# Yixin-F/better_fastlio2

Measured on NVIDIA H100. Metric: scans/s (120k-pt, 3 ESIKF iters) at 1xH100; kNN+Jacobian HBM GB/s vs peak, higher is better.
Workload: dtype f32 search/plane + f64 Jacobian/ESIKF

## Files before the change

better_fastlio2_b200/csrc/esikf_device.cuh:

```cuda
#pragma once
#include "meas_kernels.cuh"

namespace flb {

namespace dev {

constexpr int ESIKF_THREADS = 256;

__device__ __forceinline__ void qmul(const double* a, const double* b, double* r) {
  const double x = a[3] * b[0] + a[0] * b[3] + a[1] * b[2] - a[2] * b[1];
  const double y = a[3] * b[1] + a[1] * b[3] + a[2] * b[0] - a[0] * b[2];
  const double z = a[3] * b[2] + a[2] * b[3] + a[0] * b[1] - a[1] * b[0];
  const double w = a[3] * b[3] - a[0] * b[0] - a[1] * b[1] - a[2] * b[2];
  r[0] = x; r[1] = y; r[2] = z; r[3] = w;
}
__device__ __forceinline__ void rotmat(const double* q, double* R) {
  const double tx = 2 * q[0], ty = 2 * q[1], tz = 2 * q[2];
  const double twx = tx * q[3], twy = ty * q[3], twz = tz * q[3], txx = tx * q[0], txy = ty * q[0], txz = tz * q[0];
  const double tyy = ty * q[1], tyz = tz * q[1], tzz = tz * q[2];
  R[0] = 1 - (tyy + tzz); R[1] = txy - twz; R[2] = txz + twy;
  R[3] = txy + twz; R[4] = 1 - (txx + tzz); R[5] = tyz - twx;
  R[6] = txz - twy; R[7] = tyz + twx; R[8] = 1 - (txx + tyy);
}
__device__ __forceinline__ void hat(const double* v, double* H) {
// ... 172 lines not shown
  if (tid < PROJ_OUT) v = proj_row_value(M, NDOF, q, c);
  __syncthreads();
  if (tid < PROJ_OUT) M[(q.idx + q.i) * NDOF + c] = v;
  __syncthreads();
  if (tid < PROJ_OUT) v = proj_col_value(M, q, c);
  __syncthreads();
  if (tid < PROJ_OUT) M[c * NDOF + q.idx + q.i] = v;
  __syncthreads();
}
}

__global__ void k_esikf_begin(EsikfCtl* c, const double* __restrict__ stage, int* work_counts) {
  pdl_sync();
  FLB_TRACE_BEGIN(0);
  if (threadIdx.x == 0) c->t_begin = global_timer_ns();
  __shared__ double sst[26 + NDOF * NDOF + 4];
  constexpr int NPAIR = (26 + NDOF * NDOF + 4) / 2;
  const double2* st2 = reinterpret_cast<const double2*>(stage);
  for (int i = threadIdx.x; i < NPAIR; i += blockDim.x) {
    const double2 v = st2[i];
    sst[2 * i] = v.x;
    sst[2 * i + 1] = v.y;
  }
  if (threadIdx.x >= 32 && threadIdx.x < 48) work_counts[threadIdx.x - 32] = 0;
  __syncthreads();
  const double* x0 = sst;
  const double* P0 = sst + 26;
  const int n = (int)sst[26 + NDOF * NDOF];
  for (int i = threadIdx.x; i < NDOF * NDOF; i += blockDim.x) { c->Pp[i] = P0[i]; c->P[i] = P0[i]; }
  if (threadIdx.x < 26) { c->x[threadIdx.x] = x0[threadIdx.x]; c->xp[threadIdx.x] = x0[threadIdx.x]; }
  __syncthreads();
  if (threadIdx.x == 0) {
    c->it = -1; c->t = 0; c->converge = 1; c->finished = 0; c->need_host = 0; c->passes = 0; c->searches = 0;
    c->lastM = 0; c->last_res = 0.0; c->n = n; c->flg_inited = (int)sst[26 + NDOF * NDOF + 1];
    c->body = reinterpret_cast<const float4*>((unsigned long long)__double_as_longlong(sst[26 + NDOF * NDOF + 2]));
    dev::pose_from_state(c->x, c->pose);
  }
  FLB_TRACE_END(0);
}

struct StepResult {
  double x[26];
  double P[NDOF * NDOF];
  double last_res;
  int passes, searches, lastM, t, need_host, pad_;
  int counters[32];
  int cnt2[2];
// ... 281 lines not shown
```

better_fastlio2_b200/csrc/fastlio_b200.cu:

```cuda
#include "../../include/fastlio_b200.h"
#include "map_kernels.cuh"
#include "knn_kernels.cuh"
#include "frontend_kernels.cuh"
#include "meas_kernels.cuh"
#include "esikf_device.cuh"
#include "knn_tile.cuh"
#include "esikf_host.hpp"

#include <cub/device/device_scan.cuh>
#include <algorithm>
#include <chrono>
#include <climits>
#include <cstdarg>
#include <cstdio>
#include <cstdlib>
#include <cstring>
#include <new>
#include <vector>

using namespace flb;

static thread_local char g_err[512] = "";
static int set_err(const char* fmt, ...) {
  va_list ap;
// ... 33 lines not shown
template <typename T> using DevBuf = GrowBuf<T, false>;
template <typename T> using PinnedBuf = GrowBuf<T, true>;

template <typename T, bool Pinned>
static int grow(GrowBuf<T, Pinned>& b, size_t need, size_t floor) {
  if (need <= b.cap) return 0;
  b.release();
  const size_t cap = std::max(need, floor);
  void* p = nullptr;
  CU(Pinned ? cudaMallocHost(&p, cap) : cudaMalloc(&p, cap));
  b.p = static_cast<T*>(p);
  b.cap = cap;
  return 0;
}

extern "C" const char* flb_last_error(void) { return g_err; }
extern "C" const char* flb_version(void) { return "fastlio_b200 0.1 (sm_90a)"; }
extern "C" int flb_device_count(void) {
  int n = 0;
  if (cudaGetDeviceCount(&n) != cudaSuccess) { cudaGetLastError(); return 0; }
  return n;
}

static bool pdl_enabled() {
  static const bool on = [] { const char* e = getenv("FLB_PDL"); return e && atoi(e) != 0; }();
  return on;
}
template <typename... P, typename... A>
static cudaError_t launch_k(void (*kern)(P...), dim3 grid, dim3 block, size_t smem, cudaStream_t st, A&&... args) {
  cudaLaunchConfig_t cfg{};
  cfg.gridDim = grid; cfg.blockDim = block; cfg.dynamicSmemBytes = smem; cfg.stream = st;
  cudaLaunchAttribute at[1];
  at[0].id = cudaLaunchAttributeProgrammaticStreamSerialization;
  at[0].val.programmaticStreamSerializationAllowed = 1;
  cfg.attrs = at;
  cfg.numAttrs = pdl_enabled() ? 1 : 0;
  return cudaLaunchKernelEx(&cfg, kern, static_cast<P>(args)...);
}

static inline uint32_t next_pow2(uint64_t v) {
  uint32_t p = 1;
  while (p < v) p <<= 1;
  return p;
}
static inline int grid_for(int n, int threads, int max_blocks) {
  int g = (n + threads - 1) / threads;
  if (g < 1) g = 1;
  return g > max_blocks ? max_blocks : g;
}
template <typename... P>
static cudaError_t resident_ctas(void (*kern)(P...), int threads, size_t smem, int sm_count, int& out) {
  int per_sm = 0;
  const cudaError_t e = cudaOccupancyMaxActiveBlocksPerMultiprocessor(&per_sm, kern, threads, smem);
  out = std::max(per_sm, 1) * sm_count;
  return e;
}

struct flb_map {
  MapDev d{};
  flb_map_config cfg{};
// ... 71 lines not shown
  m->has_root = false;
  return 0;
}

static int absorb_range_flag(flb_map* m) {
  int e = m->h_counters[CNT_ERROR];
  if (!(e & ERR_RANGE)) return e;
  if (!m->warned_range) {
    fprintf(stderr, "[fastlio_b200] warning: point(s) outside the representable range / NaN were skipped by the map insert\n");
    m->warned_range = true;
  }
  e &= ~ERR_RANGE;
  m->h_counters[CNT_ERROR] = e;
  if (cudaMemcpyAsync(m->d.counters + CNT_ERROR, m->h_counters + CNT_ERROR, sizeof(int), cudaMemcpyHostToDevice, m->stream) == cudaSuccess)
    cudaStreamSynchronize(m->stream);
  return e;
}

static int fetch_counters(flb_map* m) {
  CU(cudaMemcpyAsync(m->h_counters, m->d.counters, sizeof(int) * CNT_COUNT, cudaMemcpyDeviceToHost, m->stream));
  CU(cudaStreamSynchronize(m->stream));
  const int e = absorb_range_flag(m);
  if (e) {
    return set_err("device map error flags 0x%x:%s%s%s%s%s", e, (e & ERR_BLOCKS_FULL) ? " block pool exhausted (raise max_blocks)" : "",
                   (e & ERR_OVF_FULL) ? " overflow pool exhausted (raise max_points)" : "", (e & ERR_HASH_FULL) ? " block hash full" : "",
                   (e & ERR_COARSE_FULL) ? " coarse hash full" : "", (e & ERR_RANGE) ? " point outside representable range / NaN" : "");
  }
  return 0;
}

extern "C" int flb_map_create(const flb_map_config* cfg, flb_map** out) {
  if (!cfg || !out) return set_err("flb_map_create: null argument");
  cudaGetLastError();
  if (!(cfg->voxel_size > 0.f)) return set_err("flb_map_create: voxel_size must be > 0");
  int ndev = flb_device_count();
  if (ndev <= 0) return set_err("flb_map_create: no CUDA device available (this library has no CPU fallback)");
  if (cfg->device < 0 || cfg->device >= ndev) return set_err("flb_map_create: bad device %d", cfg->device);
  CU(cudaSetDevice(cfg->device));
  flb_map* m = new (std::nothrow) flb_map();
  if (!m) return set_err("out of host memory");
  m->cfg = *cfg;
  if (m->cfg.max_points <= 0) m->cfg.max_points = 8 * 1024 * 1024;
  if (m->cfg.max_blocks <= 0) m->cfg.max_blocks = std::max(4096, m->cfg.max_points / 4);
  cudaDeviceProp prop;
  CU(cudaGetDeviceProperties(&prop, cfg->device));
  m->sm_count = prop.multiProcessorCount;
  CU(resident_ctas(k_knn<5>, KNN_THREADS, 0, m->sm_count, m->exact_ctas[0]));
  CU(resident_ctas(k_knn<20>, KNN_THREADS, 0, m->sm_count, m->exact_ctas[1]));
  CU(cudaStreamCreateWithFlags(&m->stream, cudaStreamNonBlocking));
  MapDev& d = m->d;
  d.ds = cfg->voxel_size;
  d.block_cap = m->cfg.max_blocks;
  d.ovf_cap = std::max(1024, m->cfg.max_points / 2);
  m->hash_cap = next_pow2((uint64_t)d.block_cap * 4);
  m->chash_cap = next_pow2(std::max<uint64_t>(1024, (uint64_t)d.block_cap / 8));
  d.hash_mask = m->hash_cap - 1;
  d.chash_mask = m->chash_cap - 1;
  int rc = 0;
  rc |= dev_alloc(m, (void**)&d.hent, sizeof(HEntry) * m->hash_cap);
  rc |= dev_alloc(m, (void**)&d.bslot, sizeof(uint32_t) * d.block_cap);
  rc |= dev_alloc(m, (void**)&d.slots, sizeof(float4) * 64 * (size_t)d.block_cap);
  rc |= dev_alloc(m, (void**)&d.ovf, sizeof(float4) * (size_t)d.ovf_cap);
  rc |= dev_alloc(m, (void**)&d.sint, sizeof(float) * 64 * (size_t)d.block_cap);
  rc |= dev_alloc(m, (void**)&d.oint, sizeof(float) * (size_t)d.ovf_cap);
  rc |= dev_alloc(m, (void**)&d.bkey, sizeof(uint64_t) * d.block_cap);
  rc |= dev_alloc(m, (void**)&d.brel, sizeof(uint64_t) * d.block_cap);
  rc |= dev_alloc(m, (void**)&d.free_blk, sizeof(uint32_t) * d.block_cap);
  rc |= dev_alloc(m, (void**)&d.free_ovf, sizeof(uint32_t) * d.ovf_cap);
  rc |= dev_alloc(m, (void**)&d.ckeys, sizeof(uint64_t) * m->chash_cap);
  rc |= dev_alloc(m, (void**)&d.cbits, sizeof(uint64_t) * 8 * (size_t)m->chash_cap);
  rc |= dev_alloc(m, (void**)&d.clist, sizeof(uint32_t) * (size_t)m->chash_cap);
  rc |= dev_alloc(m, (void**)&d.counters, sizeof(int) * CNT_COUNT);
  rc |= dev_alloc(m, (void**)&m->d_misc, sizeof(int) * 32);
  rc |= dev_alloc(m, (void**)&m->d_phase, sizeof(int) * 8);
  if (rc) { flb_map_destroy(m); return 1; }
  if (cudaMallocHost((void**)&m->h_counters, sizeof(int) * CNT_COUNT) != cudaSuccess) { flb_map_destroy(m); return set_err("cudaMallocHost failed"); }
  unsigned char ti[91], tj[91];
  int e = 0;
  for (int i = 0; i < 13; ++i) for (int j = i; j < 13; ++j) { ti[e] = (unsigned char)i; tj[e] = (unsigned char)j; ++e; }
  CU(cudaMemcpyToSymbol(c_tri_i, ti, sizeof(ti)));
  CU(cudaMemcpyToSymbol(c_tri_j, tj, sizeof(tj)));
  if (map_reset_storage(m)) { flb_map_destroy(m); return 1; }
  *out = m;
  return 0;
}

static void map_release(flb_map* m);
static void kfw_release(KfWork* w);
extern "C" void flb_map_destroy(flb_map* m) {
  if (!m) return;
  map_release(m);
}
static void map_release(flb_map* m) {
  if (--m->refs > 0) return;
  Q(cudaSetDevice(m->cfg.device));
  if (m->stream) Q(cudaStreamSynchronize(m->stream));
// ... 43 lines not shown
  return pack_records(m, st, raw.p, n, stride, off_i, off_c, dst, curv);
}

static int upload_points(flb_map* m, const void* pts, int n, int stride, int off_i = -1) {
  if (n <= 0) return 0;
  if (!pts) return set_err("null point buffer");
  if (stride < 12) return set_err("stride_bytes must be >= 12");
  if (off_i >= 0 && off_i + 4 > stride) return set_err("intensity offset %d outside the %d-byte record", off_i, stride);
  if (stride == 16 && off_i < 0) off_i = 12;
  if (grow(m->stage, sizeof(float4) * (size_t)n, sizeof(float4) << 16)) return 1;
  return upload_records(m, m->stream, m->raw, (size_t)1 << 20, pts, n, stride, off_i, -1, m->stage.p, nullptr);
}

static inline uint32_t scratch_slots(int n) { return next_pow2((uint64_t)std::max(n, 512) * 2); }

static int ensure_scratch(flb_map* m, int n) {
  const size_t need = sizeof(uint64_t) * scratch_slots(n);
  if (need <= m->skeys.cap && need <= m->sbest.cap) return 0;
  if (grow(m->skeys, need, 0) || grow(m->sbest, need, 0)) return 1;
  m->gen++;
  return 0;
}

static int ensure_worklist(flb_map* m, int n) {
  const size_t need = sizeof(int) * (size_t)n;
  if (need <= m->worklist.cap) return 0;
  if (grow(m->worklist, need, sizeof(int) << 17)) return 1;
  m->gen++;
  return 0;
}

static int maybe_rehash(flb_map* m);

static int insert_device(flb_map* m, const float4* pts, const unsigned char* cls, int n, int mode, const int* skip = nullptr,
                         const int* n_dev = nullptr, bool prefused = false, StepTail tail = StepTail{}) {
  if (n <= 0) return 0;
  const int g = grid_for(n, 256, m->sm_count * 8);
  cudaStream_t st = m->stream;
  const unsigned char* c = (mode == 2) ? cls : nullptr;
  ProfScope ps(m, FLB_K_INSERT);
  if (!prefused) {
    launch_k(k_touch_blocks, g, 256, 0, st, m->d, pts, c, (1 << 1) | (1 << 2), n, skip, n_dev);
    m->launches++;
  }
  if (mode == 1 || mode == 2) {
    const uint32_t sc = scratch_slots(n);
    if (!prefused) {
      if (ensure_scratch(m, n)) return 1;
      if (!m->scratch_clean) {
        CU(cudaMemsetAsync(m->skeys.p, 0xFF, sizeof(uint64_t) * sc, st));
// ... 113 lines not shown
  m->launches += 2;
  CU(cudaMemsetAsync(m->d.ckeys, 0xFF, sizeof(uint64_t) * m->chash_cap, st));
  CU(cudaMemsetAsync(m->d.cbits, 0, sizeof(uint64_t) * 8 * (size_t)m->chash_cap, st));
  int init[8] = {0, 0, INT_MAX, INT_MAX, INT_MAX, INT_MIN, INT_MIN, INT_MIN};
  CU(cudaMemcpyAsync(m->d.counters + CNT_KEYS_TOMB, &init[0], sizeof(int), cudaMemcpyHostToDevice, st));
  CU(cudaMemcpyAsync(m->d.counters + CNT_COARSE_USED, &init[1], sizeof(int), cudaMemcpyHostToDevice, st));
  CU(cudaMemcpyAsync(m->d.counters + CNT_CMIN_X, &init[2], sizeof(int) * 6, cudaMemcpyHostToDevice, st));
  CU(cudaStreamSynchronize(st));
  k_rehash_insert<<<grid_for(nblk, 256, m->sm_count * 8), 256, 0, st>>>(m->d, nblk);
  m->launches++;
  CU(cudaGetLastError());
  m->rehash_count++;
  return fetch_counters(m);
}

template <int K>
static int launch_knn(flb_map* m, KnnArgs a) {
  if (ensure_worklist(m, a.n)) return 1;
  a.worklist = m->worklist.p;
  if (a.stride <= 0) a.stride = a.n;
  if (!a.work_count) {
    a.work_count = m->d_misc + 12;
    a.work_ticket = m->d_misc + 13;
    CU(cudaMemsetAsync(a.work_count, 0, 2 * sizeof(int), m->stream));
  }
  launch_k(k_knn_stencil<K>, (a.n + 127) / 128, 128, 0, m->stream, a);
  launch_k(k_knn<K>, m->exact_ctas[K == 5 ? 0 : 1], KNN_THREADS, 0, m->stream, a);
  m->launches += 2;
  return 0;
}

static int ensure_outbuf(flb_map* m, int n) { return grow(m->outbuf, sizeof(float4) * (size_t)n, sizeof(float4) << 16); }

static int nearest_search_impl(flb_map* m, const float* q_xyz, int nq, int stride, int k, float max_dist, float* out_pts, int out_w,
                               float* out_d2, int* out_cnt) {
  if (!m) return set_err("null map");
  if (k < 1 || k > 20) return set_err("Nearest_Search: k must be in [1,20]");
  if (nq <= 0) return 0;
  CU(cudaSetDevice(m->cfg.device));
  if (upload_points(m, q_xyz, nq, stride)) return 1;
  const int K = k <= 5 ? 5 : 20;
  if (ensure_outbuf(m, nq * K)) return 1;
  unsigned char* dcnt = nullptr;
  float* dint = nullptr;
  CU(cudaMalloc((void**)&dcnt, nq));
  KnnArgs a;
  a.m = m->d; a.q = m->stage.p; a.n = nq; a.nbr = m->outbuf.p; a.cnt = dcnt;
  a.max_d2 = (max_dist > 0.f && max_dist < 1e18f) ? max_dist * max_dist : INFINITY;
  a.phase_stats = nullptr;
  a.ctl = nullptr; a.body = nullptr; a.stride = nq; a.work_count = nullptr;
// ... 166 lines not shown
    float ms = 0.f;
    if (cudaEventElapsedTime(&ms, r.a, r.b) != cudaSuccess) continue;
    if (r.cls >= 0 && r.cls < FLB_K_COUNT) { out->ms[r.cls] += ms; out->launches[r.cls] += r.nlaunch; out->regions[r.cls] += 1; }
  }
  int ph[8];
  CU(cudaMemcpy(ph, m->d_phase, sizeof(ph), cudaMemcpyDeviceToHost));
  for (int i = 0; i < 4; ++i) out->knn_phase[i] = ph[i];
  out->knn_chain_nodes = ph[4]; out->knn_chain_max = ph[5]; out->knn_head_candidates = ph[6];
  if (reset) { m->prof_used = 0; CU(cudaMemset(m->d_phase, 0, sizeof(int) * 8)); }
  return 0;
}

extern "C" int flb_debug_knn_bench(flb_map* m, const float* q_xyz, int nq, int stride, int variant, int iters, float* ms_per_launch,
                                   int* unresolved, float* out_d2, int* out_cnt) {
  if (!m || !q_xyz || nq <= 0 || iters <= 0) return set_err("flb_debug_knn_bench: bad argument");
  CU(cudaSetDevice(m->cfg.device));
  if (upload_points(m, q_xyz, nq, stride)) return 1;
  if (ensure_outbuf(m, nq * 5)) return 1;
  if (ensure_worklist(m, nq)) return 1;
  unsigned char* dcnt = nullptr;
  CU(cudaMalloc((void**)&dcnt, nq));
  KnnArgs a;
  a.m = m->d; a.q = m->stage.p; a.n = nq; a.nbr = m->outbuf.p; a.cnt = dcnt; a.max_d2 = INFINITY; a.phase_stats = nullptr;
  a.worklist = m->worklist.p; a.work_count = m->d_misc + 12; a.work_ticket = m->d_misc + 13; a.ctl = nullptr; a.body = nullptr; a.stride = nq;
  cudaError_t e = cudaFuncSetAttribute(k_knn_tile<5>, cudaFuncAttributeMaxDynamicSharedMemorySize, (int)sizeof(TileSmem));
  cudaEvent_t e0 = nullptr, e1 = nullptr;
  if (e == cudaSuccess) e = cudaEventCreate(&e0);
  if (e == cudaSuccess) e = cudaEventCreate(&e1);
  const int grid = (nq + 127) / 128;
  for (int it = -2; it < iters && e == cudaSuccess; ++it) {
    if (it == 0) e = cudaEventRecord(e0, m->stream);
    if (e == cudaSuccess) e = cudaMemsetAsync(a.work_count, 0, 2 * sizeof(int), m->stream);
    if (variant == 0) k_knn_stencil<5><<<grid, 128, 0, m->stream>>>(a);
    else k_knn_tile<5><<<grid, TILE_THREADS, sizeof(TileSmem), m->stream>>>(a);
    if (e == cudaSuccess) e = cudaGetLastError();
  }
  if (e == cudaSuccess) e = cudaEventRecord(e1, m->stream);
  if (e == cudaSuccess) e = cudaStreamSynchronize(m->stream);
  float ms = 0.f;
  if (e == cudaSuccess) e = cudaEventElapsedTime(&ms, e0, e1);
  if (ms_per_launch) *ms_per_launch = ms / (float)iters;
  if (e == cudaSuccess && unresolved) e = cudaMemcpy(unresolved, a.work_count, sizeof(int), cudaMemcpyDeviceToHost);
  if (e == cudaSuccess && out_d2) {
    std::vector<float4> h((size_t)nq * 5);
    e = cudaMemcpy(h.data(), m->outbuf.p, sizeof(float4) * h.size(), cudaMemcpyDeviceToHost);
    for (int i = 0; i < nq && e == cudaSuccess; ++i)
      for (int j = 0; j < 5; ++j) out_d2[(size_t)i * 5 + j] = h[(size_t)j * nq + i].w;
  }
  if (e == cudaSuccess && out_cnt) {
    std::vector<unsigned char> hc(nq);
    e = cudaMemcpy(hc.data(), dcnt, nq, cudaMemcpyDeviceToHost);
    for (int i = 0; i < nq; ++i) out_cnt[i] = hc[i];
  }
  cudaFree(dcnt);
  if (e0) cudaEventDestroy(e0);
  if (e1) cudaEventDestroy(e1);
  if (e != cudaSuccess) return set_err("flb_debug_knn_bench: %s", cudaGetErrorString(e));
  return 0;
}

struct flb_session {
// ... 425 lines not shown
      if (md12) k_esikf_pre<12><<<1, dev::ESIKF_THREADS, 0, s->side>>>(s->ctl, s->d_scr);
      else k_esikf_pre<6><<<1, dev::ESIKF_THREADS, 0, s->side>>>(s->ctl, s->d_scr);
      if (p == 0 && with_insert) {
        if (!m->capturing && ensure_scratch(m, cap)) return 1;
        const uint32_t sc = scratch_slots(cap);
        CU(cudaMemsetAsync(m->skeys.p, 0xFF, sizeof(uint64_t) * sc, s->side));
        CU(cudaMemsetAsync(m->sbest.p, 0xFF, sizeof(unsigned long long) * sc, s->side));
        CU(cudaMemsetAsync(s->d_cnt2, 0, sizeof(int) * 2, s->side));
        m->scratch_clean = true;
      }
      CU(cudaEventRecord(s->ev_join[p], s->side));
    } else {
      ProfScope ps(m, FLB_K_REDUCE);
      if (md12) k_esikf_pre<12><<<1, dev::ESIKF_THREADS, 0, st>>>(s->ctl, s->d_scr);
      else k_esikf_pre<6><<<1, dev::ESIKF_THREADS, 0, st>>>(s->ctl, s->d_scr);
    }
    m->launches++;
    {
      ProfScope ps(m, FLB_K_KNN);
      KnnArgs a;
      a.m = m->d; a.q = nullptr; a.n = cap; a.nbr = s->nbr; a.cnt = s->cnt; a.max_d2 = INFINITY;
      a.phase_stats = m->prof_on ? m->d_phase : nullptr;
      a.ctl = s->ctl; a.body = nullptr; a.stride = cap; a.work_count = p < 8 ? m->d_misc + 16 + p : nullptr; a.work_ticket = p < 8 ? m->d_misc + 24 + p : nullptr;
      if (launch_knn<5>(m, a)) return 1;
    }
    {
      ProfScope ps(m, FLB_K_RESIDUAL);
      MeasArgs ma = meas_args(s, PoseDev{}, 0);
      ma.ctl = s->ctl;
      if (s->cfg.extrinsic_est_en) launch_k(k_residual<true>, s->res_grid, meas_threads<true>(), meas_smem_bytes<true>(), st, ma);
      else launch_k(k_residual<false>, s->res_grid, meas_threads<false>(), meas_smem_bytes<false>(), st, ma);
      m->launches++;
    }
    if (overlap) CU(cudaStreamWaitEvent(st, s->ev_join[p], 0));
    {
      ProfScope ps(m, FLB_K_REDUCE);
      if (md12) launch_k(k_esikf_post<12>, 1, dev::ESIKF_THREADS, 0, st, s->ctl, (const double*)s->partial, s->res_grid, s->d_scr);
      else launch_k(k_esikf_post<6>, 1, dev::ESIKF_THREADS, 0, st, s->ctl, (const double*)s->partial, s->res_grid, s->d_scr);
      m->launches++;
    }
  }
  CU(cudaGetLastError());
  const bool tail_publish = overlap && with_insert && s->cap > 0;
  if (tail_publish) {
    CU(cudaEventRecord(s->ev_fork[8], st));
    CU(cudaStreamWaitEvent(s->side, s->ev_fork[8], 0));
// ... 377 lines not shown
```

better_fastlio2_b200/csrc/knn_kernels.cuh:

```cuda
#pragma once
#include "mask_bits.h"
#include "voxel_map.cuh"
#include <math_constants.h>

namespace flb {

constexpr unsigned FULL = 0xffffffffu;
constexpr int BLOCK_RINGS = 8;
#ifndef FLB_KNN_THREADS
#define FLB_KNN_THREADS 128
#endif
#ifndef FLB_KNN_MINB
#define FLB_KNN_MINB 4
#endif
constexpr int KNN_THREADS = FLB_KNN_THREADS;
constexpr int KNN_MIN_CTAS = FLB_KNN_MINB;

__host__ __device__ constexpr int topk_unroll(int k) { return k <= 8 ? k : 1; }

template <int K>
struct TopK {
  float d[K], x[K], y[K], z[K];
  __device__ __forceinline__ void clear() {
#pragma unroll (topk_unroll(K))
// ... 112 lines not shown
  double limit[NDOF];
  double R;
  double last_res;
  PoseDev pose;
  int max_iter, it, t, converge, finished, need_host, passes, searches, lastM, n;
  int flg_inited;
  int pad_;
  const float4* body;
  unsigned long long t_begin;
};
__device__ __forceinline__ bool ctl_pass_active(const EsikfCtl* c) { return !c->finished && c->it < c->max_iter; }

struct KnnArgs {
  MapDev m;
  const float4* q;
  int n;
  float4* nbr;
  unsigned char* cnt;
  float max_d2;
  int* phase_stats;
  int* worklist;
  int* work_count;
  int* work_ticket;
  const EsikfCtl* ctl;
  const float4* body;
  int stride;
};

__device__ __forceinline__ float box_mind2(float qx, float qy, float qz, float lx, float ly, float lz, float hx, float hy, float hz, float mg) {
  const float gx = fmaxf(fmaxf(lx - qx, qx - hx) - mg, 0.f);
  const float gy = fmaxf(fmaxf(ly - qy, qy - hy) - mg, 0.f);
  const float gz = fmaxf(fmaxf(lz - qz, qz - hz) - mg, 0.f);
  return gx * gx + gy * gy + gz * gz;
}
__device__ __forceinline__ float cover2(float qx, float qy, float qz, float lx, float ly, float lz, float hx, float hy, float hz, float mg) {
  float c = fminf(fminf(fminf(qx - lx, hx - qx), fminf(qy - ly, hy - qy)), fminf(qz - lz, hz - qz)) - mg;
  return c > 0.f ? c * c : 0.f;
}

constexpr int EXACT_RINGS = 8;
constexpr int CAND_CAP = 512;

struct ExactSmem {
  unsigned cand[KNN_THREADS / 32][CAND_CAP];
  unsigned long long cbits[KNN_THREADS / 32][27 * 8];
};
// ... 232 lines not shown
#pragma unroll 1
        for (int base = 0; base < ncs; base += 32) {
          int cs;
          const float md = cell_md(base + lane, cs);
          const bool go = md > level && md < CUDART_INF_F && (wcount < K || md <= wthr) && md <= lim;
          unsigned todo = __ballot_sync(FULL, go);
          if (!todo) continue;
          while (todo) {
            const int c = __ffs(todo) - 1;
            todo &= todo - 1;
            scan_coarse_cell<K>(m, cand, cb, __shfl_sync(FULL, cs, c), lane, wqx, wqy, wqz, cvx, cvy, cvz, wcount == K, wthr, lim, mg, tw);
          }
          wcount = warp_merge<K>(tw, FULL, lane, lane, wd_, wx, wy, wz, wthr);
        }
      }
    }
    if (lane < K) nbr[(size_t)lane * stride + qi] = make_float4(wx, wy, wz, wd_);
    if (lane == 0) {
      cnt[qi] = (unsigned char)wcount;
      if (phase_stats) atomicAdd(&phase_stats[phase], 1);
    }
}

template <int K>
__global__ void __launch_bounds__(KNN_THREADS, KNN_MIN_CTAS) k_knn(KnnArgs a) {
  pdl_sync();
  __shared__ ExactSmem sm;
  const MapDev& m = a.m;
  const int lane = threadIdx.x & 31, wid = threadIdx.x >> 5;
  const float ds = m.ds;
  const float lim = a.max_d2;
  unsigned* cand = sm.cand[wid];
  unsigned long long* cb = sm.cbits[wid];
  FLB_TRACE_BEGIN(3 * 8 + (a.ctl ? a.ctl->it + 1 : 0));
  if (a.ctl && !(ctl_pass_active(a.ctl) && a.ctl->converge)) return;
  const int nwork = *a.work_count;
  const int nwarps = (int)(gridDim.x * (blockDim.x >> 5));
  int w = (int)(blockIdx.x * (blockDim.x >> 5)) + wid;
  for (;; ) {
    if (w >= nwork) break;
    const int i = a.worklist[w];
    const float4 q4 = a.ctl ? body_to_world(a.ctl->pose, __ldg(&a.ctl->body[i])) : __ldg(&a.q[i]);
    const float qx = q4.x, qy = q4.y, qz = q4.z;
    TopK<K> t;
    t.clear();
    float rd = CUDART_INF_F, rx = CUDART_NAN_F, ry = CUDART_NAN_F, rz = CUDART_NAN_F, thr = CUDART_INF_F;
    int gcount = a.cnt[i];
    if (lane < gcount) {
      const float4 sd = a.nbr[(size_t)lane * a.stride + i];
      rd = sd.w; rx = sd.x; ry = sd.y; rz = sd.z;
      t.d[0] = rd; t.x[0] = rx; t.y[0] = ry; t.z[0] = rz;
    }
    {
      const float dk = __shfl_sync(FULL, rd, K - 1);
      thr = gcount == K ? dk : CUDART_INF_F;
    }
    const int cvx = voxel_of(qx, ds), cvy = voxel_of(qy, ds), cvz = voxel_of(qz, ds);
    const float mg = 1e-3f * ds + 4.8e-7f * (fabsf(qx) + fabsf(qy) + fabsf(qz));
    const int qbx = cvx >> 2, qby = cvy >> 2, qbz = cvz >> 2;
    const int qcx = qbx >> 3, qcy = qby >> 3, qcz = qbz >> 3;
    const float bs4 = 4.f * ds;
    bool done = false;
    FLB_DBG_CLOCK(e0);
    int dbg_rings = 0;
    (void)dbg_rings;
#ifdef FLB_TRACE
    long long ph_probe = 0, ph_merge = 0, ph_mark = clock64();
    const long long ph_seed = ph_mark - e0;
#define KPH(acc) { const long long now_ = clock64(); acc += now_ - ph_mark; ph_mark = now_; }
#else
#define KPH(acc)
#endif
// ... 37 lines not shown
    if (done) {
      if (lane < K) a.nbr[(size_t)lane * a.stride + i] = make_float4(rx, ry, rz, rd);
      if (lane == 0) {
        a.cnt[i] = (unsigned char)gcount;
        if (a.phase_stats) atomicAdd(&a.phase_stats[1], 1);
      }
    }
#ifdef FLB_TRACE
    if (lane == 0 && a.ctl && a.ctl->it == -1) {
      const long long e1 = clock64();
      FLB_DBG_ADD(16, 1); FLB_DBG_ADD(17, e1 - e0); FLB_DBG_MAX(18, e1 - e0); FLB_DBG_ADD(18 + min(dbg_rings, 6), 1);
      FLB_DBG_ADD(25, done ? 0 : 1);
      FLB_DBG_ADD(58 + (int)min((e1 - e0) >> 13, 5ll), 1);
      FLB_DBG_ADD(32, ph_seed); FLB_DBG_ADD(33, ph_probe); FLB_DBG_ADD(36, ph_merge);
    }
#endif
    if (!done) {
      __syncwarp();
      warp_finish_coarse<K>(m, cand, cb, a.nbr, a.cnt, a.phase_stats, a.stride, lim, i, qx, qy, qz, gcount, thr, rd, rx, ry, rz);
    }
    if (lane == 0) w = nwarps + atomicAdd(a.work_ticket, 1);
    w = __shfl_sync(FULL, w, 0);
  }
  FLB_TRACE_END(3 * 8 + (a.ctl ? a.ctl->it + 1 : 0));
}

template <int K>
struct TopKId {
  float d[K];
  unsigned id[K];
  __device__ __forceinline__ void clear() {
#pragma unroll
    for (int j = 0; j < K; ++j) { d[j] = CUDART_INF_F; id[j] = 0u; }
  }
  __device__ __forceinline__ void insert(float dd, unsigned pid) {
    bool c[K];
#pragma unroll
    for (int j = 0; j < K; ++j) c[j] = dd < d[j];
#pragma unroll
    for (int j = K - 1; j > 0; --j) {
      d[j] = c[j - 1] ? d[j - 1] : (c[j] ? dd : d[j]);
      id[j] = c[j - 1] ? id[j - 1] : (c[j] ? pid : id[j]);
    }
    d[0] = c[0] ? dd : d[0];
    id[0] = c[0] ? pid : id[0];
  }
};
// ... 118 lines not shown
          const int vb = (vx >> 2) | ((vy >> 2) << 1) | ((vz >> 2) << 2);
          pid[u] = (unsigned)sm.blk[vb][tid] * 64u + (unsigned)((vx & 3) | ((vy & 3) << 2) | ((vz & 3) << 4));
          e[u] = __ldg(&m.slots[pid[u]]);
        }
      }
#pragma unroll
      for (int u = 0; u < 4; ++u) {
        if (base + u < ns) {
          float dd = sqdist(qx, qy, qz, e[u].x, e[u].y, e[u].z);
          if (dd <= lim && dd < t.d[K - 1]) t.insert(dd, pid[u]);
          ++n_head;
          walk_chain(m, __float_as_int(e[u].w), [&](const float4 o, int c) {
            ++n_chain;
            const float d2 = sqdist(qx, qy, qz, o.x, o.y, o.z);
            if (d2 <= lim && d2 < t.d[K - 1]) t.insert(d2, 0x80000000u | (unsigned)c);
          });
        }
      }
    }
  }
}

template <int K>
__global__ void __launch_bounds__(STENCIL_THREADS, 7) k_knn_stencil(KnnArgs a) {
  pdl_sync();
  __shared__ StencilSmem sm;
  const MapDev& m = a.m;
  const int tid = threadIdx.x;
  const int i = blockIdx.x * blockDim.x + tid;
  FLB_TRACE_BEGIN(2 * 8 + (a.ctl ? a.ctl->it + 1 : 0));
  if (a.ctl && !(ctl_pass_active(a.ctl) && a.ctl->converge)) return;
  if (i >= (a.ctl ? a.ctl->n : a.n)) return;
  const float ds = m.ds;
  const float lim = a.max_d2;
  const float4 q4 = a.ctl ? body_to_world(a.ctl->pose, __ldg(&a.ctl->body[i])) : __ldg(&a.q[i]);
  const float qx = q4.x, qy = q4.y, qz = q4.z;
  const float qlim = 4.0e6f * ds;
  TopKId<K> t;
  t.clear();
  bool done = false;
  FLB_DBG_CLOCK(w0);
  bool dbg_fallback = false;
  (void)dbg_fallback;
  if (fabsf(qx) < qlim && fabsf(qy) < qlim && fabsf(qz) < qlim) {
    const int cvx = voxel_of(qx, ds), cvy = voxel_of(qy, ds), cvz = voxel_of(qz, ds);
    const int bbx = (cvx - 2) >> 2, bby = (cvy - 2) >> 2, bbz = (cvz - 2) >> 2;
    const float mg = 1e-3f * ds + 4.8e-7f * (fabsf(qx) + fabsf(qy) + fabsf(qz));
    const int ox = (cvx - 2) & 3, oy = (cvy - 2) & 3, oz = (cvz - 2) & 3;
    const unsigned ax5 = 31u << ox, ay5 = 31u << oy, az5 = 31u << oz;
    const unsigned ix = 14u << ox, iy = 14u << oy, iz = 14u << oz;
#pragma unroll
    for (int j = 0; j < 5; ++j) {
      const float lx = (float)(cvx - 2 + j) * ds, ly = (float)(cvy - 2 + j) * ds, lz = (float)(cvz - 2 + j) * ds;
      const float gx = fmaxf(fmaxf(lx - qx, qx - (lx + ds)) - mg, 0.f);
      const float gy = fmaxf(fmaxf(ly - qy, qy - (ly + ds)) - mg, 0.f);
// ... 57 lines not shown
    }
    const float cov = cover2(qx, qy, qz, (float)(cvx - 2) * ds, (float)(cvy - 2) * ds, (float)(cvz - 2) * ds,
                             (float)(cvx + 3) * ds, (float)(cvy + 3) * ds, (float)(cvz + 3) * ds, mg);
    done = (t.d[K - 1] < CUDART_INF_F && t.d[K - 1] < cov) || cov > lim;
  } else {
    done = true;
  }
  int c = 0;
#pragma unroll
  for (int r = 0; r < K; ++r) {
    const bool ok = t.d[r] < CUDART_INF_F;
    c += ok ? 1 : 0;
    float4 o = make_float4(CUDART_NAN_F, CUDART_NAN_F, CUDART_NAN_F, CUDART_INF_F);
    if (ok) {
      const float4 e = (t.id[r] & 0x80000000u) ? __ldg(&m.ovf[t.id[r] & 0x7FFFFFFFu]) : __ldg(&m.slots[t.id[r]]);
      o = make_float4(e.x, e.y, e.z, t.d[r]);
    }
    a.nbr[(size_t)r * a.stride + i] = o;
  }
  a.cnt[i] = (unsigned char)c;
  if (done) {
    if (a.phase_stats) atomicAdd(&a.phase_stats[0], 1);
  } else {
    a.worklist[atomicAdd(a.work_count, 1)] = i;
  }
  FLB_TRACE_END(2 * 8 + (a.ctl ? a.ctl->it + 1 : 0));
}

__global__ void k_transform(PoseDev s, const float4* __restrict__ body, float4* __restrict__ world, int n) {
  for (int i = blockIdx.x * blockDim.x + threadIdx.x; i < n; i += gridDim.x * blockDim.x) world[i] = body_to_world(s, body[i]);
}

}
```

better_fastlio2_b200/csrc/knn_tile.cuh:

```cuda
#pragma once
#include "knn_kernels.cuh"

namespace flb {

constexpr int TILE_THREADS = 128;
constexpr int TILE_SLOTS = 256;
constexpr int TILE_CAP = 40;
constexpr int TILE_PROBE = 24;

struct __align__(128) TileSmem {
  float4 tile[TILE_CAP][64];
  unsigned long long keys[TILE_SLOTS];
  unsigned long long tmask[TILE_SLOTS];
  int tblk[TILE_SLOTS];
  short ttile[TILE_SLOTS];
  unsigned long long mbar;
  int ntile;
  unsigned short slot[8][TILE_THREADS];
  int blk[8][TILE_THREADS];
  short tix[8][TILE_THREADS];
  unsigned long long c5[8][TILE_THREADS];
  float gap[15][TILE_THREADS];
  unsigned xy3[4][TILE_THREADS];
  unsigned z3[4][TILE_THREADS];
// ... 174 lines not shown
        }
      }
    } else {
      tile_pass<K, true>(m, sm, tid, qx, qy, qz, lim, t);
    }
    const float cov = cover2(qx, qy, qz, (float)(cvx - 2) * ds, (float)(cvy - 2) * ds, (float)(cvz - 2) * ds,
                             (float)(cvx + 3) * ds, (float)(cvy + 3) * ds, (float)(cvz + 3) * ds, mg);
    done = (t.d[K - 1] < CUDART_INF_F && t.d[K - 1] < cov) || cov > lim;
  }
  if (!valid) return;
  int c = 0;
#pragma unroll
  for (int r = 0; r < K; ++r) {
    const bool ok = t.d[r] < CUDART_INF_F;
    c += ok ? 1 : 0;
    float4 o = make_float4(CUDART_NAN_F, CUDART_NAN_F, CUDART_NAN_F, CUDART_INF_F);
    if (ok) {
      const float4 e = (t.id[r] & 0x80000000u) ? __ldg(&m.ovf[t.id[r] & 0x7FFFFFFFu]) : tile_point(m, sm, tid, (int)(t.id[r] >> 6), (int)(t.id[r] & 63u));
      o = make_float4(e.x, e.y, e.z, t.d[r]);
    }
    a.nbr[(size_t)r * a.stride + i] = o;
  }
  a.cnt[i] = (unsigned char)c;
  if (!done) a.worklist[atomicAdd(a.work_count, 1)] = i;
}

}
```

better_fastlio2_b200/csrc/trace.cuh:

```cuda
#pragma once
#ifdef FLB_TRACE
namespace flb {
constexpr int TRACE_SLOTS = 128;
constexpr int TRACE_PHASES = 96;
struct TraceRec { unsigned long long t0, t1; };
__device__ TraceRec g_trace[TRACE_SLOTS];
__device__ long long g_phase_clk[TRACE_PHASES];
__device__ __forceinline__ unsigned long long gtimer() {
  unsigned long long t;
  asm volatile("mov.u64 %0, %%globaltimer;" : "=l"(t));
  return t;
}
__device__ __forceinline__ void trace_mark(int slot, bool begin) {
  if (threadIdx.x == 0) {
    const unsigned long long t = gtimer();
    if (begin) atomicMin(&g_trace[slot].t0, t);
    else atomicMax(&g_trace[slot].t1, t);
  }
}
constexpr int TRACE_DBG = 64;
__device__ unsigned long long g_dbg[TRACE_DBG];
__device__ __forceinline__ void dbg_add(int idx, unsigned long long v) { atomicAdd(&g_dbg[idx], v); }
__device__ __forceinline__ void dbg_max(int idx, unsigned long long v) { atomicMax(&g_dbg[idx], v); }
__device__ __forceinline__ void trace_phase(int idx) {
  if (threadIdx.x == 0 && idx < TRACE_PHASES) g_phase_clk[idx] = clock64();
}
}
#define FLB_TRACE_BEGIN(slot) flb::trace_mark((slot), true)
#define FLB_TRACE_END(slot) flb::trace_mark((slot), false)
#define FLB_TRACE_PHASE(idx) flb::trace_phase(idx)
#define FLB_DBG_ADD(idx, v) flb::dbg_add((idx), (unsigned long long)(v))
#define FLB_DBG_MAX(idx, v) flb::dbg_max((idx), (unsigned long long)(v))
#define FLB_DBG_CLOCK(var) const long long var = clock64()
#else
#define FLB_TRACE_BEGIN(slot)
#define FLB_TRACE_END(slot)
#define FLB_TRACE_PHASE(idx)
#define FLB_DBG_ADD(idx, v)
#define FLB_DBG_MAX(idx, v)
#define FLB_DBG_CLOCK(var)
#endif
```

better_fastlio2_b200/csrc/voxel_map.cuh:

```cuda
#pragma once
#include <cuda_runtime.h>
#include <stdint.h>
#include "trace.cuh"

namespace flb {

__device__ __forceinline__ unsigned long long global_timer_ns() {
  unsigned long long t;
  asm volatile("mov.u64 %0, %%globaltimer;" : "=l"(t));
  return t;
}
__device__ __forceinline__ void pdl_sync() {
  asm volatile("griddepcontrol.wait;" ::: "memory");
  asm volatile("griddepcontrol.launch_dependents;" ::: "memory");
}

constexpr uint64_t KEY_EMPTY = 0xFFFFFFFFFFFFFFFFull;
constexpr uint64_t KEY_TOMB = 0xFFFFFFFFFFFFFFFEull;
constexpr int COORD_BIAS = 1 << 20;

enum Counter : int {
  CNT_BLK_BUMP = 0,
  CNT_BLK_FREE,
  CNT_OVF_BUMP,
  CNT_OVF_FREE,
  CNT_VALID,
  CNT_KEYS_USED,
  CNT_KEYS_TOMB,
  CNT_COARSE_USED,
  CNT_ERROR,
  CNT_SCRATCH0,
  CNT_SCRATCH1,
  CNT_SCRATCH2,
  CNT_CMIN_X, CNT_CMIN_Y, CNT_CMIN_Z,
  CNT_CMAX_X, CNT_CMAX_Y, CNT_CMAX_Z,
  CNT_COUNT = 32
};
enum DevError : int { ERR_BLOCKS_FULL = 1, ERR_OVF_FULL = 2, ERR_HASH_FULL = 4, ERR_COARSE_FULL = 8, ERR_RANGE = 16 };

struct __align__(32) HEntry {
  uint64_t key;
  uint32_t val;
  uint32_t pad;
  uint64_t mask;
  uint64_t pad2;
};

struct MapDev {
  HEntry* hent;
  uint32_t* bslot;
  float4* slots;
  float* sint;
  float4* ovf;
  float* oint;
  uint64_t* bkey;
  uint64_t* brel;
  uint32_t* free_blk;
  uint32_t* free_ovf;
  uint64_t* ckeys;
  uint64_t* cbits;
  uint32_t* clist;
// ... 109 lines not shown
```

Baseline: 3977.

## Overlap exact k-NN kernel with stencil via PDL and streaming work-list handoff

The exact k-NN kernel is now always launched with programmatic dependent launch and no longer waits for the stencil kernel to finish. Warps instead poll work-list slots that the stencil publishes with release stores. The last stencil block writes end sentinels for every exact warp, and the slots are pre-filled with an empty marker and reset after use. The goal is to hide the exact search's launch latency and tail behind the stencil pass. The cost is spin-waiting warps occupying SMs, a timeout error path, and a risk of deadlock if the exact CTAs become resident before stencil blocks can be scheduled.

```diff
diff --git a/better_fastlio2_b200/csrc/esikf_device.cuh b/better_fastlio2_b200/csrc/esikf_device.cuh
--- a/better_fastlio2_b200/csrc/esikf_device.cuh
+++ b/better_fastlio2_b200/csrc/esikf_device.cuh
@@ -218,7 +218,7 @@
     sst[2 * i] = v.x;
     sst[2 * i + 1] = v.y;
   }
-  if (threadIdx.x >= 32 && threadIdx.x < 48) work_counts[threadIdx.x - 32] = 0;
+  if (threadIdx.x >= 32 && threadIdx.x < 56) work_counts[threadIdx.x - 32] = 0;
   __syncthreads();
   const double* x0 = sst;
   const double* P0 = sst + 26;
diff --git a/better_fastlio2_b200/csrc/fastlio_b200.cu b/better_fastlio2_b200/csrc/fastlio_b200.cu
--- a/better_fastlio2_b200/csrc/fastlio_b200.cu
+++ b/better_fastlio2_b200/csrc/fastlio_b200.cu
@@ -79,20 +79,24 @@
   return n;
 }
 
-static bool pdl_enabled() {
-  static const bool on = [] { const char* e = getenv("FLB_PDL"); return e && atoi(e) != 0; }();
-  return on;
-}
 template <typename... P, typename... A>
-static cudaError_t launch_k(void (*kern)(P...), dim3 grid, dim3 block, size_t smem, cudaStream_t st, A&&... args) {
+static cudaError_t launch_kx(bool programmatic, void (*kern)(P...), dim3 grid, dim3 block, size_t smem, cudaStream_t st, A&&... args) {
   cudaLaunchConfig_t cfg{};
   cfg.gridDim = grid; cfg.blockDim = block; cfg.dynamicSmemBytes = smem; cfg.stream = st;
   cudaLaunchAttribute at[1];
   at[0].id = cudaLaunchAttributeProgrammaticStreamSerialization;
   at[0].val.programmaticStreamSerializationAllowed = 1;
   cfg.attrs = at;
-  cfg.numAttrs = pdl_enabled() ? 1 : 0;
+  cfg.numAttrs = programmatic ? 1 : 0;
   return cudaLaunchKernelEx(&cfg, kern, static_cast<P>(args)...);
+}
+static bool pdl_enabled() {
+  static const bool on = [] { const char* e = getenv("FLB_PDL"); return e && atoi(e) != 0; }();
+  return on;
+}
+template <typename... P, typename... A>
+static cudaError_t launch_k(void (*kern)(P...), dim3 grid, dim3 block, size_t smem, cudaStream_t st, A&&... args) {
+  return launch_kx(pdl_enabled(), kern, grid, block, smem, st, static_cast<A&&>(args)...);
 }
 
 static inline uint32_t next_pow2(uint64_t v) {
@@ -210,9 +214,10 @@
   CU(cudaStreamSynchronize(m->stream));
   const int e = absorb_range_flag(m);
   if (e) {
-    return set_err("device map error flags 0x%x:%s%s%s%s%s", e, (e & ERR_BLOCKS_FULL) ? " block pool exhausted (raise max_blocks)" : "",
+    return set_err("device map error flags 0x%x:%s%s%s%s%s%s", e, (e & ERR_BLOCKS_FULL) ? " block pool exhausted (raise max_blocks)" : "",
                    (e & ERR_OVF_FULL) ? " overflow pool exhausted (raise max_points)" : "", (e & ERR_HASH_FULL) ? " block hash full" : "",
-                   (e & ERR_COARSE_FULL) ? " coarse hash full" : "", (e & ERR_RANGE) ? " point outside representable range / NaN" : "");
+                   (e & ERR_COARSE_FULL) ? " coarse hash full" : "", (e & ERR_RANGE) ? " point outside representable range / NaN" : "",
+                   (e & ERR_KNN_STALL) ? " k-NN work-list wait timed out" : "");
   }
   return 0;
 }
@@ -259,7 +264,7 @@
   rc |= dev_alloc(m, (void**)&d.cbits, sizeof(uint64_t) * 8 * (size_t)m->chash_cap);
   rc |= dev_alloc(m, (void**)&d.clist, sizeof(uint32_t) * (size_t)m->chash_cap);
   rc |= dev_alloc(m, (void**)&d.counters, sizeof(int) * CNT_COUNT);
-  rc |= dev_alloc(m, (void**)&m->d_misc, sizeof(int) * 32);
+  rc |= dev_alloc(m, (void**)&m->d_misc, sizeof(int) * 48);
   rc |= dev_alloc(m, (void**)&m->d_phase, sizeof(int) * 8);
   if (rc) { flb_map_destroy(m); return 1; }
   if (cudaMallocHost((void**)&m->h_counters, sizeof(int) * CNT_COUNT) != cudaSuccess) { flb_map_destroy(m); return set_err("cudaMallocHost failed"); }
@@ -349,10 +354,13 @@
   return 0;
 }
 
+static int exact_warps(const flb_map* m, int K) { return m->exact_ctas[K == 5 ? 0 : 1] * (KNN_THREADS / 32); }
+
 static int ensure_worklist(flb_map* m, int n) {
-  const size_t need = sizeof(int) * (size_t)n;
+  const size_t need = sizeof(int) * ((size_t)n + std::max(exact_warps(m, 5), exact_warps(m, 20)));
   if (need <= m->worklist.cap) return 0;
   if (grow(m->worklist, need, sizeof(int) << 17)) return 1;
+  CU(cudaMemsetAsync(m->worklist.p, 0xFF, m->worklist.cap, m->stream));
   m->gen++;
   return 0;
 }
@@ -512,10 +520,12 @@
   if (!a.work_count) {
     a.work_count = m->d_misc + 12;
     a.work_ticket = m->d_misc + 13;
-    CU(cudaMemsetAsync(a.work_count, 0, 2 * sizeof(int), m->stream));
-  }
+    a.stencil_done = m->d_misc + 14;
+    CU(cudaMemsetAsync(a.work_count, 0, 3 * sizeof(int), m->stream));
+  }
+  a.exact_warps = exact_warps(m, K);
   launch_k(k_knn_stencil<K>, (a.n + 127) / 128, 128, 0, m->stream, a);
-  launch_k(k_knn<K>, m->exact_ctas[K == 5 ? 0 : 1], KNN_THREADS, 0, m->stream, a);
+  launch_kx(true, k_knn<K>, m->exact_ctas[K == 5 ? 0 : 1], KNN_THREADS, 0, m->stream, a);
   m->launches += 2;
   return 0;
 }
@@ -728,7 +738,8 @@
   CU(cudaMalloc((void**)&dcnt, nq));
   KnnArgs a;
   a.m = m->d; a.q = m->stage.p; a.n = nq; a.nbr = m->outbuf.p; a.cnt = dcnt; a.max_d2 = INFINITY; a.phase_stats = nullptr;
-  a.worklist = m->worklist.p; a.work_count = m->d_misc + 12; a.work_ticket = m->d_misc + 13; a.ctl = nullptr; a.body = nullptr; a.stride = nq;
+  a.worklist = m->worklist.p; a.work_count = m->d_misc + 12; a.work_ticket = m->d_misc + 13; a.stencil_done = m->d_misc + 14;
+  a.exact_warps = exact_warps(m, 5); a.ctl = nullptr; a.body = nullptr; a.stride = nq;
   cudaError_t e = cudaFuncSetAttribute(k_knn_tile<5>, cudaFuncAttributeMaxDynamicSharedMemorySize, (int)sizeof(TileSmem));
   cudaEvent_t e0 = nullptr, e1 = nullptr;
   if (e == cudaSuccess) e = cudaEventCreate(&e0);
@@ -736,13 +747,14 @@
   const int grid = (nq + 127) / 128;
   for (int it = -2; it < iters && e == cudaSuccess; ++it) {
     if (it == 0) e = cudaEventRecord(e0, m->stream);
-    if (e == cudaSuccess) e = cudaMemsetAsync(a.work_count, 0, 2 * sizeof(int), m->stream);
+    if (e == cudaSuccess) e = cudaMemsetAsync(a.work_count, 0, 3 * sizeof(int), m->stream);
     if (variant == 0) k_knn_stencil<5><<<grid, 128, 0, m->stream>>>(a);
     else k_knn_tile<5><<<grid, TILE_THREADS, sizeof(TileSmem), m->stream>>>(a);
     if (e == cudaSuccess) e = cudaGetLastError();
   }
   if (e == cudaSuccess) e = cudaEventRecord(e1, m->stream);
   if (e == cudaSuccess) e = cudaStreamSynchronize(m->stream);
+  if (e == cudaSuccess) e = cudaMemsetAsync(m->worklist.p, 0xFF, m->worklist.cap, m->stream);
   float ms = 0.f;
   if (e == cudaSuccess) e = cudaEventElapsedTime(&ms, e0, e1);
   if (ms_per_launch) *ms_per_launch = ms / (float)iters;
@@ -1214,6 +1226,7 @@
       a.m = m->d; a.q = nullptr; a.n = cap; a.nbr = s->nbr; a.cnt = s->cnt; a.max_d2 = INFINITY;
       a.phase_stats = m->prof_on ? m->d_phase : nullptr;
       a.ctl = s->ctl; a.body = nullptr; a.stride = cap; a.work_count = p < 8 ? m->d_misc + 16 + p : nullptr; a.work_ticket = p < 8 ? m->d_misc + 24 + p : nullptr;
+      a.stencil_done = p < 8 ? m->d_misc + 32 + p : nullptr;
       if (launch_knn<5>(m, a)) return 1;
     }
     {
diff --git a/better_fastlio2_b200/csrc/knn_kernels.cuh b/better_fastlio2_b200/csrc/knn_kernels.cuh
--- a/better_fastlio2_b200/csrc/knn_kernels.cuh
+++ b/better_fastlio2_b200/csrc/knn_kernels.cuh
@@ -158,6 +158,8 @@
   int* worklist;
   int* work_count;
   int* work_ticket;
+  int* stencil_done;
+  int exact_warps;
   const EsikfCtl* ctl;
   const float4* body;
   int stride;
@@ -436,9 +438,38 @@
     }
 }
 
+constexpr int WORK_EMPTY = -1;
+constexpr int WORK_END = -2;
+constexpr unsigned long long KNN_WAIT_NS = 1000000000ull;
+
+__device__ __forceinline__ int worklist_take(const KnnArgs& a, int w, int lane) {
+  int v = WORK_EMPTY;
+  if (lane == 0) {
+    v = ld_relaxed(&a.worklist[w]);
+    if (v == WORK_EMPTY) {
+      const unsigned long long t0 = global_timer_ns();
+      unsigned ns = 32;
+      do {
+        __nanosleep(ns);
+        ns = min(2u * ns, 512u);
+        v = ld_relaxed(&a.worklist[w]);
+        if (v == WORK_EMPTY && global_timer_ns() - t0 > KNN_WAIT_NS) {
+          atomicOr(&a.m.counters[CNT_ERROR], ERR_KNN_STALL);
+          v = WORK_END;
+        }
+      } while (v == WORK_EMPTY);
+    }
+    if (v >= 0) v = ld_acquire(&a.worklist[w]);
+    a.worklist[w] = WORK_EMPTY;
+  }
+  v = __shfl_sync(FULL, v, 0);
+  __syncwarp();
+  return v == WORK_END ? -1 : v;
+}
+
 template <int K>
 __global__ void __launch_bounds__(KNN_THREADS, KNN_MIN_CTAS) k_knn(KnnArgs a) {
-  pdl_sync();
+  pdl_trigger();
   __shared__ ExactSmem sm;
   const MapDev& m = a.m;
   const int lane = threadIdx.x & 31, wid = threadIdx.x >> 5;
@@ -446,22 +477,31 @@
   const float lim = a.max_d2;
   unsigned* cand = sm.cand[wid];
   unsigned long long* cb = sm.cbits[wid];
-  FLB_TRACE_BEGIN(3 * 8 + (a.ctl ? a.ctl->it + 1 : 0));
-  if (a.ctl && !(ctl_pass_active(a.ctl) && a.ctl->converge)) return;
-  const int nwork = *a.work_count;
+  const bool active = !(a.ctl && !(ctl_pass_active(a.ctl) && a.ctl->converge)) && (a.ctl ? a.ctl->n : a.n) > 0;
+#ifdef FLB_TRACE
+  const int tslot = 3 * 8 + (a.ctl ? a.ctl->it + 1 : 0);
+  bool first_take = true;
+#endif
   const int nwarps = (int)(gridDim.x * (blockDim.x >> 5));
   int w = (int)(blockIdx.x * (blockDim.x >> 5)) + wid;
-  for (;; ) {
-    if (w >= nwork) break;
-    const int i = a.worklist[w];
+  for (; active; ) {
+    const int i = worklist_take(a, w, lane);
+    if (i < 0) break;
+#ifdef FLB_TRACE
+    if (lane == 0) {
+      if (first_take) FLB_TRACE_STAMP(tslot, true);
+      if (a.ctl && a.ctl->it == -1) FLB_TRACE_HIST(80, 2 * 8);
+    }
+    first_take = false;
+#endif
     const float4 q4 = a.ctl ? body_to_world(a.ctl->pose, __ldg(&a.ctl->body[i])) : __ldg(&a.q[i]);
     const float qx = q4.x, qy = q4.y, qz = q4.z;
     TopK<K> t;
     t.clear();
     float rd = CUDART_INF_F, rx = CUDART_NAN_F, ry = CUDART_NAN_F, rz = CUDART_NAN_F, thr = CUDART_INF_F;
-    int gcount = a.cnt[i];
+    int gcount = __ldcg(&a.cnt[i]);
     if (lane < gcount) {
-      const float4 sd = a.nbr[(size_t)lane * a.stride + i];
+      const float4 sd = __ldcg(&a.nbr[(size_t)lane * a.stride + i]);
       rd = sd.w; rx = sd.x; ry = sd.y; rz = sd.z;
       t.d[0] = rd; t.x[0] = rx; t.y[0] = ry; t.z[0] = rz;
     }
@@ -545,7 +585,10 @@
     if (lane == 0) w = nwarps + atomicAdd(a.work_ticket, 1);
     w = __shfl_sync(FULL, w, 0);
   }
-  FLB_TRACE_END(3 * 8 + (a.ctl ? a.ctl->it + 1 : 0));
+  pdl_wait();
+#ifdef FLB_TRACE
+  if (lane == 0 && active) FLB_TRACE_STAMP(tslot, false);
+#endif
 }
 
 template <int K>
@@ -710,15 +753,8 @@
 }
 
 template <int K>
-__global__ void __launch_bounds__(STENCIL_THREADS, 7) k_knn_stencil(KnnArgs a) {
-  pdl_sync();
-  __shared__ StencilSmem sm;
+__device__ __forceinline__ void stencil_query(const KnnArgs& a, StencilSmem& sm, int tid, int i) {
   const MapDev& m = a.m;
-  const int tid = threadIdx.x;
-  const int i = blockIdx.x * blockDim.x + tid;
-  FLB_TRACE_BEGIN(2 * 8 + (a.ctl ? a.ctl->it + 1 : 0));
-  if (a.ctl && !(ctl_pass_active(a.ctl) && a.ctl->converge)) return;
-  if (i >= (a.ctl ? a.ctl->n : a.n)) return;
   const float ds = m.ds;
   const float lim = a.max_d2;
   const float4 q4 = a.ctl ? body_to_world(a.ctl->pose, __ldg(&a.ctl->body[i])) : __ldg(&a.q[i]);
@@ -822,7 +858,34 @@
   if (done) {
     if (a.phase_stats) atomicAdd(&a.phase_stats[0], 1);
   } else {
-    a.worklist[atomicAdd(a.work_count, 1)] = i;
+    st_release(&a.worklist[atomicAdd(a.work_count, 1)], i);
+#ifdef FLB_TRACE
+    if (a.ctl && a.ctl->it == -1) FLB_TRACE_HIST(64, 2 * 8);
+#endif
+  }
+}
+
+template <int K>
+__global__ void __launch_bounds__(STENCIL_THREADS, 7) k_knn_stencil(KnnArgs a) {
+  pdl_sync();
+  __shared__ StencilSmem sm;
+  const int tid = threadIdx.x;
+  FLB_TRACE_BEGIN(2 * 8 + (a.ctl ? a.ctl->it + 1 : 0));
+  if (a.ctl && !(ctl_pass_active(a.ctl) && a.ctl->converge)) return;
+  const int n = a.ctl ? a.ctl->n : a.n;
+  if ((int)blockIdx.x * STENCIL_THREADS >= n) return;
+  const int i = blockIdx.x * STENCIL_THREADS + tid;
+  if (i < n) stencil_query<K>(a, sm, tid, i);
+  __syncthreads();
+  int last = 0;
+  if (tid == 0) {
+    const int nq = a.ctl ? a.ctl->n : a.n;
+    last = atom_add_release(a.stencil_done, 1) == (nq + STENCIL_THREADS - 1) / STENCIL_THREADS - 1;
+    if (last) __threadfence();
+  }
+  if (__syncthreads_or(last)) {
+    const int nw = ld_relaxed(a.work_count);
+    for (int j = tid; j < a.exact_warps; j += STENCIL_THREADS) st_relaxed(&a.worklist[nw + j], WORK_END);
   }
   FLB_TRACE_END(2 * 8 + (a.ctl ? a.ctl->it + 1 : 0));
 }
diff --git a/better_fastlio2_b200/csrc/knn_tile.cuh b/better_fastlio2_b200/csrc/knn_tile.cuh
--- a/better_fastlio2_b200/csrc/knn_tile.cuh
+++ b/better_fastlio2_b200/csrc/knn_tile.cuh
@@ -220,7 +220,7 @@
     a.nbr[(size_t)r * a.stride + i] = o;
   }
   a.cnt[i] = (unsigned char)c;
-  if (!done) a.worklist[atomicAdd(a.work_count, 1)] = i;
-}
-
-}
+  if (!done) st_release(&a.worklist[atomicAdd(a.work_count, 1)], i);
+}
+
+}
diff --git a/better_fastlio2_b200/csrc/trace.cuh b/better_fastlio2_b200/csrc/trace.cuh
--- a/better_fastlio2_b200/csrc/trace.cuh
+++ b/better_fastlio2_b200/csrc/trace.cuh
@@ -18,7 +18,17 @@
     else atomicMax(&g_trace[slot].t1, t);
   }
 }
-constexpr int TRACE_DBG = 64;
+__device__ __forceinline__ void trace_stamp(int slot, bool begin) {
+  const unsigned long long t = gtimer();
+  if (begin) atomicMin(&g_trace[slot].t0, t);
+  else atomicMax(&g_trace[slot].t1, t);
+}
+__device__ __forceinline__ int trace_bucket_since(int slot) {
+  const unsigned long long t0 = *(volatile unsigned long long*)&g_trace[slot].t0;
+  const unsigned long long t = gtimer();
+  return t > t0 ? (int)min((t - t0) / 4000ull, 15ull) : 0;
+}
+constexpr int TRACE_DBG = 128;
 __device__ unsigned long long g_dbg[TRACE_DBG];
 __device__ __forceinline__ void dbg_add(int idx, unsigned long long v) { atomicAdd(&g_dbg[idx], v); }
 __device__ __forceinline__ void dbg_max(int idx, unsigned long long v) { atomicMax(&g_dbg[idx], v); }
@@ -32,6 +42,8 @@
 #define FLB_DBG_ADD(idx, v) flb::dbg_add((idx), (unsigned long long)(v))
 #define FLB_DBG_MAX(idx, v) flb::dbg_max((idx), (unsigned long long)(v))
 #define FLB_DBG_CLOCK(var) const long long var = clock64()
+#define FLB_TRACE_STAMP(slot, begin) flb::trace_stamp((slot), (begin))
+#define FLB_TRACE_HIST(idx0, slot) flb::dbg_add((idx0) + flb::trace_bucket_since(slot), 1)
 #else
 #define FLB_TRACE_BEGIN(slot)
 #define FLB_TRACE_END(slot)
@@ -39,4 +51,6 @@
 #define FLB_DBG_ADD(idx, v)
 #define FLB_DBG_MAX(idx, v)
 #define FLB_DBG_CLOCK(var)
+#define FLB_TRACE_STAMP(slot, begin)
+#define FLB_TRACE_HIST(idx0, slot)
 #endif
diff --git a/better_fastlio2_b200/csrc/voxel_map.cuh b/better_fastlio2_b200/csrc/voxel_map.cuh
--- a/better_fastlio2_b200/csrc/voxel_map.cuh
+++ b/better_fastlio2_b200/csrc/voxel_map.cuh
@@ -10,9 +10,28 @@
   asm volatile("mov.u64 %0, %%globaltimer;" : "=l"(t));
   return t;
 }
+__device__ __forceinline__ void pdl_wait() { asm volatile("griddepcontrol.wait;" ::: "memory"); }
+__device__ __forceinline__ void pdl_trigger() { asm volatile("griddepcontrol.launch_dependents;" ::: "memory"); }
 __device__ __forceinline__ void pdl_sync() {
-  asm volatile("griddepcontrol.wait;" ::: "memory");
-  asm volatile("griddepcontrol.launch_dependents;" ::: "memory");
+  pdl_wait();
+  pdl_trigger();
+}
+__device__ __forceinline__ void st_release(int* p, int v) { asm volatile("st.release.gpu.global.s32 [%0], %1;" ::"l"(p), "r"(v) : "memory"); }
+__device__ __forceinline__ void st_relaxed(int* p, int v) { asm volatile("st.relaxed.gpu.global.s32 [%0], %1;" ::"l"(p), "r"(v) : "memory"); }
+__device__ __forceinline__ int ld_relaxed(const int* p) {
+  int v;
+  asm volatile("ld.relaxed.gpu.global.s32 %0, [%1];" : "=r"(v) : "l"(p) : "memory");
+  return v;
+}
+__device__ __forceinline__ int ld_acquire(const int* p) {
+  int v;
+  asm volatile("ld.acquire.gpu.global.s32 %0, [%1];" : "=r"(v) : "l"(p) : "memory");
+  return v;
+}
+__device__ __forceinline__ int atom_add_release(int* p, int v) {
+  int old;
+  asm volatile("atom.release.gpu.global.add.s32 %0, [%1], %2;" : "=r"(old) : "l"(p), "r"(v) : "memory");
+  return old;
 }
 
 constexpr uint64_t KEY_EMPTY = 0xFFFFFFFFFFFFFFFFull;
@@ -36,7 +55,7 @@
   CNT_CMAX_X, CNT_CMAX_Y, CNT_CMAX_Z,
   CNT_COUNT = 32
 };
-enum DevError : int { ERR_BLOCKS_FULL = 1, ERR_OVF_FULL = 2, ERR_HASH_FULL = 4, ERR_COARSE_FULL = 8, ERR_RANGE = 16 };
+enum DevError : int { ERR_BLOCKS_FULL = 1, ERR_OVF_FULL = 2, ERR_HASH_FULL = 4, ERR_COARSE_FULL = 8, ERR_RANGE = 16, ERR_KNN_STALL = 32 };
 
 struct __align__(32) HEntry {
   uint64_t key;
```

Result: faster. 4098, median of 6 (+3.0%).
